# scale-lab/MTLoRA

Hardware: AMD Instinct MI355X
Metric: images/sec (train step) Swin-T/448 r=64 4-task (higher is better)
Workload: dtype bf16; 1 GPU; BASELINE configs[1]: Swin-T 448, 4 tasks (semseg,normals,sal,human_parts), r_shared=64 r_task=4 scale4; train step (fwd+loss+bwd+clip+AdamW), dropout .05, drop_path .2; per_gpu_batch=32, global_batch=32, img_size=448, parallelism=dp1, trainable_params=8344634, allreduce_bytes=0

## Files before the change

include/mtlora_hip.h:

```cpp
#ifndef MTLORA_HIP_H
#define MTLORA_HIP_H

#include <stdint.h>

#ifdef __cplusplus
extern "C" {
#endif

#define MTLORA_ABI_VERSION 9
#define MTLORA_MAX_TASKS 8

typedef enum mtlora_dtype {
    MTLORA_F32 = 0,
    MTLORA_BF16 = 1,
    MTLORA_F16 = 2
} mtlora_dtype;

typedef enum mtlora_status {
    MTLORA_OK = 0,
    MTLORA_ERR_DTYPE = -1,
    MTLORA_ERR_SHAPE = -2,
    MTLORA_ERR_ALIGN = -3,
    MTLORA_ERR_NULL = -4,
    MTLORA_ERR_WORKSPACE = -5,
    MTLORA_ERR_HIP = -6,
    MTLORA_ERR_UNSUPPORTED = -7
} mtlora_status;

int mtlora_version(void);
const char* mtlora_error_string(int status);

int mtlora_roll_and_window_partition_forward(const void* image, void* windows, int64_t B, int64_t H, int64_t W,
// ... 134 lines not shown
                                          void* const* d_branch, float* dgamma, float* dbeta, const float* scale, int64_t B,
                                          int64_t M, int64_t C, int x_dtype, int dy_dtype, void* scratch, int64_t scratch_bytes,
                                          const void* const* dx_addend, int merge_h, int merge_w, void* stream);

int mtlora_residual_layernorm_multi_fwd(int n, const void* shortcut, const void* const* branch, const float* scale, int64_t B,
                                        const float* gamma, const float* beta, void* const* x_new, void* const* y,
                                        float* const* mean, float* const* rstd, int64_t M, int64_t C, float eps, int x_dtype,
                                        int y_dtype, void* stream);
int mtlora_residual_layernorm_multi_bwd(int n, const void* const* dy, const void* const* x_new, const float* gamma,
                                        const float* const* mean, const float* const* rstd, const void* const* dx_addend,
                                        void* d_shortcut, void* const* d_branch, float* dgamma, float* dbeta, const float* scale,
                                        int64_t B, int64_t M, int64_t C, int x_dtype, int dy_dtype, void* scratch,
                                        int64_t scratch_bytes, void* stream);

int64_t mtlora_bn_scratch_bytes(int64_t R, int64_t C, int dtype);
int mtlora_bn_relu_fwd(const void* x, const float* gamma, const float* beta, float* running_mean, float* running_var,
                       float momentum, float eps, int relu, void* y, float* save_mean, float* save_rstd,
                       float* save_scale, float* save_shift, int64_t R, int64_t C, int dtype, void* scratch,
                       int64_t scratch_bytes, void* stream);
int mtlora_bn_relu_bwd(const void* dy, const void* x, const float* save_mean, const float* save_rstd,
                       const float* save_scale, const float* save_shift, int relu, void* dx, float* dgamma, float* dbeta,
                       int64_t R, int64_t C, int dtype, void* scratch, int64_t scratch_bytes, void* stream);

int mtlora_residual_droppath_fwd(int n, const void* const* res, const void* const* y, void* const* out,
                                 const float* scale, int64_t M, int64_t C, int64_t B, int res_dtype, int y_dtype,
                                 void* stream);
int mtlora_residual_droppath_bwd(int n, const void* const* g, void* const* dy, void* dres, const float* scale,
                                 int64_t M, int64_t C, int64_t B, int res_dtype, int y_dtype, void* stream);

int64_t mtlora_upsample_loss_partials(int64_t B, int h, int w, int scale);
int mtlora_upsample_loss(int kind, const void* low, const float* label, const float* stat, void* dlow, float* partials,
                         int64_t B, int h, int w, int C, int scale, int dtype, float ignore_index, void* stream);

int mtlora_upsample_metrics_sizes(int kind, int64_t B, int h, int w, int C, int scale, int64_t* n_int64,
                                  int64_t* n_float_partials);
int mtlora_upsample_metrics(int kind, const void* low, const float* label, const float* stat, int64_t* counts,
                            float* fpartials, int64_t B, int h, int w, int C, int scale, int dtype, float ignore_index,
                            void* stream);

int64_t mtlora_colsum_scratch_bytes(int64_t M, int64_t N);
int mtlora_colsum(const void* x, int64_t M, int64_t N, int dtype, float* out, void* scratch, int64_t scratch_bytes, void* stream);
int64_t mtlora_label_stat_scratch_bytes(int64_t n);
int mtlora_label_stat(const float* label, int64_t n, int kind, float ignore_index, float* out, void* scratch,
                      int64_t scratch_bytes, void* stream);

int mtlora_upsample_cl_fwd(const void* coarse, void* fine, int64_t B, int h, int w, int C, int scale, int64_t ld_fine,
// ... 68 lines not shown
```

mtlora_amd/_lib.py:

```python
from __future__ import annotations

import ctypes
import os
from ctypes import POINTER, Structure, c_char_p, c_float, c_int, c_int32, c_int64, c_uint64, c_void_p

import torch

MAX_TASKS = 8
ABI_VERSION = 9
F32, BF16, F16 = 0, 1, 2
_DT = {torch.float32: F32, torch.bfloat16: BF16, torch.float16: F16}

_HERE = os.path.dirname(os.path.abspath(__file__))
LIB_PATH = os.path.join(_HERE, "csrc", "libmtlora_hip.so")


class LinearDesc(Structure):
    _fields_ = [("M", c_int64), ("K", c_int64), ("N", c_int64), ("dtype", c_int32), ("mode", c_int32),
                ("T", c_int32), ("r_s", c_int32), ("r_t", c_int32 * MAX_TASKS), ("scale_s", c_float),
                ("scale_t", c_float * MAX_TASKS), ("has_x_tasks", c_int32), ("dropout_p", c_float),
                ("seed", c_uint64), ("seed_offset", c_void_p), ("bwd_phase", c_int32),
                ("sel_stream", c_int32), ("sel_dense", c_int32), ("sel_tn", c_int32), ("sel_projk", c_int32),
                ("max_cu", c_int32), ("packed", c_void_p),
                ("hid", c_int32), ("hid_pad_", c_int32), ("hid_ptr", c_void_p)]


HID_FWD_BASE, HID_P_GIVEN, HID_Q_GIVEN = 1, 2, 4


class AttnDesc(Structure):
    _fields_ = [("B", c_int64), ("H", c_int32), ("W", c_int32), ("window_size", c_int32), ("shift", c_int32),
                ("num_heads", c_int32), ("head_dim", c_int32), ("image_layout", c_int32), ("dtype", c_int32),
# ... 90 lines not shown
                                                      c_void_p]),
    "mtlora_residual_layernorm_streams_bwd": (c_int, [c_int, POINTER(c_void_p), POINTER(c_void_p), c_void_p, POINTER(c_void_p),
                                                      POINTER(c_void_p), POINTER(c_void_p), POINTER(c_void_p), c_void_p, c_void_p,
                                                      c_void_p, c_int64, c_int64, c_int64, c_int, c_int, c_void_p, c_int64,
                                                      POINTER(c_void_p), c_int, c_int, c_void_p]),
    "mtlora_residual_layernorm_multi_fwd": (c_int, [c_int, c_void_p, POINTER(c_void_p), c_void_p, c_int64, c_void_p, c_void_p,
                                                    POINTER(c_void_p), POINTER(c_void_p), POINTER(c_void_p), POINTER(c_void_p),
                                                    c_int64, c_int64, c_float, c_int, c_int, c_void_p]),
    "mtlora_residual_layernorm_multi_bwd": (c_int, [c_int, POINTER(c_void_p), POINTER(c_void_p), c_void_p, POINTER(c_void_p),
                                                    POINTER(c_void_p), POINTER(c_void_p), c_void_p, POINTER(c_void_p), c_void_p,
                                                    c_void_p, c_void_p, c_int64, c_int64, c_int64, c_int, c_int, c_void_p, c_int64,
                                                    c_void_p]),
    "mtlora_residual_layernorm_bwd": (c_int, [c_void_p, c_void_p, c_void_p, c_void_p, c_void_p, c_void_p, c_void_p, c_void_p,
                                              c_void_p, c_void_p, c_int64, c_int64, c_int64, c_int, c_int, c_void_p, c_int64,
                                              c_void_p, c_void_p]),
    "mtlora_layernorm_bwd": (c_int, [c_void_p, c_void_p, c_void_p, c_void_p, c_void_p, c_void_p, c_void_p, c_void_p,
                                     c_int64, c_int64, c_int, c_int, c_void_p, c_int64, c_void_p, c_int, c_int, c_void_p]),
    "mtlora_bn_scratch_bytes": (c_int64, [c_int64, c_int64, c_int]),
    "mtlora_bn_relu_fwd": (c_int, [c_void_p, c_void_p, c_void_p, c_void_p, c_void_p, c_float, c_float, c_int, c_void_p,
                                   c_void_p, c_void_p, c_void_p, c_void_p, c_int64, c_int64, c_int, c_void_p, c_int64,
                                   c_void_p]),
    "mtlora_bn_relu_bwd": (c_int, [c_void_p, c_void_p, c_void_p, c_void_p, c_void_p, c_void_p, c_int, c_void_p, c_void_p,
                                   c_void_p, c_int64, c_int64, c_int, c_void_p, c_int64, c_void_p]),
    "mtlora_residual_droppath_fwd": (c_int, [c_int, POINTER(c_void_p), POINTER(c_void_p), POINTER(c_void_p), c_void_p,
                                             c_int64, c_int64, c_int64, c_int, c_int, c_void_p]),
    "mtlora_residual_droppath_bwd": (c_int, [c_int, POINTER(c_void_p), POINTER(c_void_p), c_void_p, c_void_p, c_int64,
                                             c_int64, c_int64, c_int, c_int, c_void_p]),
    "mtlora_upsample_loss_partials": (c_int64, [c_int64, c_int, c_int, c_int]),
    "mtlora_colsum_scratch_bytes": (c_int64, [c_int64, c_int64]),
    "mtlora_colsum": (c_int, [c_void_p, c_int64, c_int64, c_int, c_void_p, c_void_p, c_int64, c_void_p]),
    "mtlora_label_stat_scratch_bytes": (c_int64, [c_int64]),
    "mtlora_label_stat": (c_int, [c_void_p, c_int64, c_int, c_float, c_void_p, c_void_p, c_int64, c_void_p]),
    "mtlora_upsample_loss": (c_int, [c_int, c_void_p, c_void_p, c_void_p, c_void_p, c_void_p, c_int64, c_int, c_int, c_int,
                                     c_int, c_int, ctypes.c_float, c_void_p]),
    "mtlora_upsample_metrics_sizes": (c_int, [c_int, c_int64, c_int, c_int, c_int, c_int, POINTER(c_int64), POINTER(c_int64)]),
    "mtlora_upsample_metrics": (c_int, [c_int, c_void_p, c_void_p, c_void_p, c_void_p, c_void_p, c_int64, c_int, c_int, c_int,
                                        c_int, c_int, ctypes.c_float, c_void_p]),
    "mtlora_upsample_cl_fwd": (c_int, [c_void_p, c_void_p, c_int64, c_int, c_int, c_int, c_int, c_int64, c_int, c_void_p]),
    "mtlora_upsample_cl_bwd": (c_int, [c_void_p, c_void_p, c_int64, c_int, c_int, c_int, c_int, c_int64, c_int, c_void_p]),
    "mtlora_block_save_bytes": (c_int64, [POINTER(BlockDesc)]),
    "mtlora_block_fwd_tmp_bytes": (c_int64, [POINTER(BlockDesc)]),
    "mtlora_block_bwd_scratch_bytes": (c_int64, [POINTER(BlockDesc)]),
    "mtlora_block_fwd": (c_int, [POINTER(BlockDesc), POINTER(BlockParams), c_void_p, c_void_p, c_void_p, c_void_p, c_void_p, c_int64,
                                 c_void_p, c_int64, c_void_p]),
    "mtlora_block_bwd": (c_int, [POINTER(BlockDesc), POINTER(BlockParams), c_void_p, c_void_p, c_void_p, c_void_p, c_void_p, c_void_p,
                                 c_int64, POINTER(BlockGrads), c_void_p, c_int64, c_int, c_void_p]),
# ... 84 lines not shown
```

mtlora_amd/csrc/build.py:

```python
import os
import subprocess
import sys
from concurrent.futures import ThreadPoolExecutor

HERE = os.path.dirname(os.path.abspath(__file__))
SOURCES = ["window_process.hip", "linear.hip", "attention.hip", "glue.hip", "loss.hip", "metrics.hip", "upsample.hip", "reduce.hip", "selftest.hip", "block.hip", "hid.hip"]
LIB = os.path.join(HERE, "libmtlora_hip.so")
FLAGS = ["--offload-arch=gfx950", "-O3", "-std=c++17", "-fPIC", "-Wno-unused-value", "-Wno-unused-result"]
if os.environ.get("MTLORA_ABLATE") == "1":
    FLAGS.append("-DMTL_NT_ABLATE=1")


def _hipcc():
    for c in (os.environ.get("HIPCC"), "/opt/rocm/bin/hipcc", "hipcc"):
        if c and (os.path.isabs(c) and os.path.exists(c) or not os.path.isabs(c)):
            return c
    return "hipcc"


def _stale(target, deps):
    if not os.path.exists(target):
        return True
    t = os.path.getmtime(target)
    return any(os.path.getmtime(d) > t for d in deps)


def build(force=False, verbose=True):
    hdrs = [os.path.join(HERE, f) for f in sorted(os.listdir(HERE)) if f.endswith(".h")]
    hdrs.append(os.path.join(HERE, "..", "..", "include", "mtlora_hip.h"))
# ... 25 lines not shown
```

mtlora_amd/csrc/glue.hip:

```cpp
#include "common.h"
#include "internal.h"

namespace {

constexpr int LN_MAXV = 8;

template <typename T>
__device__ __forceinline__ void ld_vec(const T* p, float (&f)[8]);
template <>
__device__ __forceinline__ void ld_vec<float>(const float* p, float (&f)[8]) {
    f32x4 v = *reinterpret_cast<const f32x4*>(p);
    f[0] = v[0];
    f[1] = v[1];
    f[2] = v[2];
    f[3] = v[3];
}
template <>
__device__ __forceinline__ void ld_vec<bf16>(const bf16* p, float (&f)[8]) {
    Vec16<bf16> v = mtl_ld16<bf16>(p);
#pragma unroll
    for (int e = 0; e < 8; ++e) f[e] = (float)v.e[e];
}
template <>
__device__ __forceinline__ void ld_vec<f16>(const f16* p, float (&f)[8]) {
// ... 1651 lines not shown
        MtlProfScope prof(PK_BN, (double)R * C * es * 2, s);
        if (dtype == MTLORA_F32)
            hipLaunchKernelGGL((k_bn_colsum<float, true>), dim3(p.nblk), dim3(threads), lds, s, p);
        else if (dtype == MTLORA_F16)
            hipLaunchKernelGGL((k_bn_colsum<f16, true>), dim3(p.nblk), dim3(threads), lds, s, p);
        else
            hipLaunchKernelGGL((k_bn_colsum<bf16, true>), dim3(p.nblk), dim3(threads), lds, s, p);
    }
    hipLaunchKernelGGL(k_bn_bwd_finalize, dim3((unsigned)mtl_ceil_div(C, 64)), dim3(64 * BN_FW), 0, s, p);
    {
        MtlProfScope prof(PK_BN, (double)R * C * es * 3, s);
        if (dtype == MTLORA_F32)
            hipLaunchKernelGGL((k_bn_apply<float, true>), dim3(apply_blocks), dim3(threads), 0, s, p);
        else if (dtype == MTLORA_F16)
            hipLaunchKernelGGL((k_bn_apply<f16, true>), dim3(apply_blocks), dim3(threads), 0, s, p);
        else
            hipLaunchKernelGGL((k_bn_apply<bf16, true>), dim3(apply_blocks), dim3(threads), 0, s, p);
    }
    MTL_CHECK_LAUNCH();
    return MTLORA_OK;
}
}

namespace {

struct ResParams {
    const void* res[MTLORA_MAX_TASKS + 1];
    const void* y[MTLORA_MAX_TASKS + 1];
    void* out[MTLORA_MAX_TASKS + 1];
    void* dres;
    const float* scale;
    int64_t M;
    int C, n, B;
    int64_t rows_per_sample;
};

template <typename TR, typename TY>
__global__ __launch_bounds__(256) void k_residual_fwd(const ResParams p) {
    const int64_t nvec = p.M * p.C / 8;
    const int k = blockIdx.y;
    const TR* res = reinterpret_cast<const TR*>(p.res[k]);
    const TY* y = reinterpret_cast<const TY*>(p.y[k]);
    TR* out = reinterpret_cast<TR*>(p.out[k]);
    for (int64_t i = (int64_t)blockIdx.x * 256 + threadIdx.x; i < nvec; i += (int64_t)gridDim.x * 256) {
        const int64_t row = (i * 8) / p.C;
        const float s = p.scale ? p.scale[(int64_t)k * p.B + row / p.rows_per_sample] : 1.f;
// ... 161 lines not shown
```

mtlora_amd/csrc/internal.h:

```cpp
#pragma once
#include <stdint.h>

#include "../../include/mtlora_hip.h"

#define MTL_INTERNAL extern "C" __attribute__((visibility("hidden")))

MTL_INTERNAL int mtli_layernorm_bwd(const void* dy, const void* x, const float* gamma, const float* mean, const float* rstd, void* dx,
                                    float* dgamma, float* dbeta, int64_t M, int64_t C, int x_dtype, int dy_dtype, void* scratch,
                                    int64_t scratch_bytes, const void* dx_addend, int phase, void* stream);
MTL_INTERNAL int mtli_residual_layernorm_bwd(const void* dy, const void* x_new, const float* gamma, const float* mean, const float* rstd,
                                             void* d_shortcut, void* d_branch, float* dgamma, float* dbeta, const float* scale,
                                             int64_t B, int64_t M, int64_t C, int x_dtype, int dy_dtype, void* scratch,
                                             int64_t scratch_bytes, const void* dx_addend, int phase, void* stream);

struct HidLaunch;
struct HidParams;
struct HidRedParams;
MTL_INTERNAL void mtli_hid_launch(const HidLaunch* L, const HidParams* q, void* stream);
MTL_INTERNAL void mtli_hid_rows_finish(int dtype, const float* rowpart, int n_chunk, int64_t M, int nt, const float* alpha, const int* off,
                                       void* out, int ldo, void* stream);
MTL_INTERNAL void mtli_hid_reduce(const HidRedParams* r, int64_t per, void* stream);
```

mtlora_amd/functional.py:

```python
from __future__ import annotations

import ctypes
import os
from dataclasses import dataclass, field
from typing import List, Optional, Sequence, Tuple

import torch

from . import _lib as L

_seed_counter = 0


_seed_offset: Optional[torch.Tensor] = None


def set_seed_offset(t: Optional[torch.Tensor]) -> None:
    global _seed_offset
    if t is not None and not (t.is_cuda and t.dtype == torch.int64 and t.numel() == 1):
        raise RuntimeError("mtlora_amd: the seed offset must be a CUDA int64 tensor with one element")
    _seed_offset = t


_factor_stream: Optional["torch.cuda.Stream"] = None
# ... 1115 lines not shown
                                    float(eps), int(relu), L.ptr(y), L.ptr(saves[0]), L.ptr(saves[1]), L.ptr(saves[2]),
                                    L.ptr(saves[3]), R, C, L.dtype_code(x), L.ptr(scratch), sb, L.stream_ptr())
        L.check(st, "mtlora_bn_relu_fwd")
        ctx.save_for_backward(x, saves)
        ctx.relu = relu
        return y

    @staticmethod
    def backward(ctx, dy):
        x, saves = ctx.saved_tensors
        R, C = x.shape
        dy = dy.to(x.dtype).contiguous()
        lib = L.lib()
        sb = lib.mtlora_bn_scratch_bytes(R, C, L.dtype_code(x))
        scratch = torch.empty(sb, dtype=torch.uint8, device=x.device)
        dx = torch.empty_like(x)
        dg = torch.empty(C, dtype=torch.float32, device=x.device)
        db = torch.empty(C, dtype=torch.float32, device=x.device)
        st = lib.mtlora_bn_relu_bwd(L.ptr(dy), L.ptr(x), L.ptr(saves[0]), L.ptr(saves[1]), L.ptr(saves[2]), L.ptr(saves[3]),
                                    int(ctx.relu), L.ptr(dx), L.ptr(dg), L.ptr(db), R, C, L.dtype_code(x), L.ptr(scratch), sb,
                                    L.stream_ptr())
        L.check(st, "mtlora_bn_relu_bwd")
        return dx, dg, db, None, None, None, None, None


class ResidualDropPathFn(torch.autograd.Function):

    @staticmethod
    def forward(ctx, scale, shared: bool, n: int, *tensors):
        nres = 1 if shared else n
        res, ys = list(tensors[:nres]), list(tensors[nres:nres + n])
        L.require_gpu(*res, *ys)
        B = res[0].shape[0]
        C = res[0].shape[-1]
        M = res[0].numel() // C
        res_c = [r.contiguous() for r in res]
        ys_c = [y.contiguous() for y in ys]
        outs = [torch.empty_like(res_c[0]) for _ in range(n)]
        rlist = res_c * n if shared else res_c
        st = L.lib().mtlora_residual_droppath_fwd(n, L.ptr_array9(rlist), L.ptr_array9(ys_c), L.ptr_array9(outs), L.ptr(scale),
                                                  M, C, B, L.dtype_code(res_c[0]), L.dtype_code(ys_c[0]), L.stream_ptr())
        L.check(st, "mtlora_residual_droppath_fwd")
        ctx.cfg = (shared, n, M, C, B, res_c[0].dtype, ys_c[0].dtype, res_c[0].shape)
        ctx.save_for_backward(scale)
        ctx.set_materialize_grads(False)
        return tuple(outs)
# ... 586 lines not shown
```

mtlora_amd/mtl_harness.py:

```python
from __future__ import annotations

import contextlib
import ctypes
import os
from typing import Dict, List, Mapping, Optional, Sequence

import torch
import torch.nn as nn
import torch.nn.functional as F

from . import functional as Fn
from .functional import BatchNormReluFn, UpsampleLossFn
from .lora import MTLoRALinear, mark_only_lora_as_trainable
from .swin_transformer_mtlora import SwinTransformerMTLoRA

NUM_OUTPUT = {"semseg": 21, "normals": 3, "sal": 1, "human_parts": 7, "depth": 1, "edge": 1}
EDGE_POS_WEIGHT = 0.95
NYUD4 = ("semseg", "depth", "normals", "edge")
NYUD_NUM_OUTPUT = {"semseg": 40}
LOSS_WEIGHTS = {"depth": 1.0, "semseg": 1.0, "human_parts": 2.0, "sal": 5.0, "edge": 50.0, "normals": 10.0}


def is_synthetic_task(t: str) -> bool:
    return len(t) >= 2 and t[0] == "t" and t[1:].isdigit()
# ... 69 lines not shown

def _streams_allowed() -> bool:
    return _GRAPH_STREAMS or not torch.cuda.is_current_stream_capturing()


class Downsampler(nn.Module):

    def __init__(self, dims, channels, input_res, bias=False, enabled=True):
        super().__init__()
        self.dims, self.input_res, self.enabled = dims, input_res, enabled
        if enabled:
            for i, (d, c) in enumerate(zip(dims, channels)):
                setattr(self, f"downsample_{i}", nn.Conv2d(d, c, 1, bias=bias))

    def forward(self, feats):
        maps = []
        for i, (f, r, d) in enumerate(zip(feats, self.input_res, self.dims)):
            if self.enabled:
                conv = getattr(self, f"downsample_{i}")
                B_, L_, _ = f.shape
                f = Fn.linear_big_m(f.reshape(B_ * L_, d), conv.weight.view(conv.out_channels, d), conv.bias).view(B_, L_, -1)
            maps.append(f.view(-1, r, r, f.shape[-1]).permute(0, 3, 1, 2))
        return maps


class HighResolutionHead(nn.Module):

    def __init__(self, backbone_channels, num_outputs):
        super().__init__()
        c = sum(backbone_channels)
        self.last_layer = nn.Sequential(nn.Conv2d(c, 4 * c, 1), nn.BatchNorm2d(4 * c, momentum=0.1),
                                        nn.ReLU(inplace=False), nn.Conv2d(4 * c, num_outputs, 1))

    def forward(self, x, channels_last_out: bool = False):
        B, _, Hh, Ww = x[0].shape
        c0, bn, _, c3 = self.last_layer
        w2d = c0.weight.view(c0.out_channels, c0.in_channels)
        xc = [m.permute(0, 2, 3, 1) for m in x]
        chans = [t.shape[3] for t in xc]
        if (x[0].is_cuda and all(t.is_contiguous() for t in xc) and all(c % 4 == 0 for c in chans[1:])
                and len({t.dtype for t in xc}) == 1 and xc[0].dtype in (torch.float32, torch.bfloat16)
                and all(Hh % t.shape[1] == 0 and Ww % t.shape[2] == 0 and Hh // t.shape[1] == Ww // t.shape[2] for t in xc)):
            t = Fn.ConcatUpsampleFn.apply(*xc)
            offs, ld = Fn.ConcatUpsampleFn.layout(chans)
            col_idx = None
            if ld != w2d.shape[1]:
                key = (tuple(offs), tuple(chans), w2d.device)
                if getattr(self, "_col_key", None) != key:
                    self._col_idx = torch.cat([torch.arange(o, o + c) for o, c in zip(offs, chans)]).to(w2d.device)
                    self._col_key = key
                col_idx = self._col_idx
        else:
            cat = torch.cat([x[0]] + [F.interpolate(m, (Hh, Ww), mode="bilinear") for m in x[1:]], 1)
            t = cat.permute(0, 2, 3, 1).reshape(B * Hh * Ww, cat.shape[1])
            col_idx = None
        h = Fn.linear_big_m(t, w2d, c0.bias, feeds_batchnorm=bn.training, col_index=col_idx)
        if bn.training and bn.track_running_stats and bn.num_batches_tracked is not None:
            bn.num_batches_tracked.add_(1)
        if bn.training and h.is_cuda and h.dtype in (torch.float32, torch.bfloat16, torch.float16) and h.shape[1] % 8 == 0:
            h = BatchNormReluFn.apply(h, bn.weight, bn.bias, bn.running_mean, bn.running_var, bn.momentum, bn.eps,
                                      getattr(self, "relu", True))
        else:
            h = F.batch_norm(h, bn.running_mean, bn.running_var, bn.weight, bn.bias, bn.training or not bn.track_running_stats,
                             bn.momentum, bn.eps)
            if getattr(self, "relu", True):
                h = F.relu(h)
        w3, b3, nc = c3.weight.view(c3.out_channels, c3.in_channels), c3.bias, c3.out_channels
        o = Fn.linear_big_m(h, w3, b3, pad_rows=(8 - nc % 8) if (h.is_cuda and nc % 8) else 0)
        o = (o if o.shape[1] == nc else o[:, :nc].contiguous()).view(B, Hh, Ww, nc)
        return o if channels_last_out else o.permute(0, 3, 1, 2)


class DecoderGroup(nn.Module):
    def __init__(self, tasks, num_outputs, channels, out_size):
        super().__init__()
        self.tasks, self.out_size = tasks, out_size
        self.decoders = nn.ModuleDict({t: HighResolutionHead(channels, num_outputs[t]) for t in tasks})

    def forward(self, x, upsample: bool = True, tasks=None):
        tasks = self.tasks if tasks is None else tasks
        if not upsample:
            return {t: self.decoders[t](x[t], channels_last_out=True) for t in tasks}
        return {t: F.interpolate(self.decoders[t](x[t]), self.out_size, mode="bilinear") for t in tasks}


class MultiTaskSwin(nn.Module):

    def __init__(self, backbone: SwinTransformerMTLoRA, tasks: Sequence[str], num_outputs: Mapping[str, int] = NUM_OUTPUT,
                 decoder_channels=(18, 36, 72, 144)):
        super().__init__()
# ... 423 lines not shown
```

Before: 1156 images/sec.

## Fuse head BatchNorm+ReLU with final 1x1 conv into custom MFMA kernels

Adds a fused head-tail path that computes BN statistics, then applies BN+ReLU on the fly while doing the small final projection with MFMA, so the normalized activation is never written out. Backward is split into a stats kernel (dgamma/dbeta, dW3, db3, BN correction terms) and an apply kernel that recomputes the BN+ReLU output and produces dz directly. This is meant to remove the materialized BN output tensor and its extra read/write traffic at large M (B*448*448/16 rows with 4C channels). It adds new kernels with per-wave slab loops and grid capped at the CU count, and it falls back to the old path when hooks are present or shapes are unsupported.

Result: slower. 1126 images/sec (-2.6%).

```diff
diff --git a/include/mtlora_hip.h b/include/mtlora_hip.h
--- a/include/mtlora_hip.h
+++ b/include/mtlora_hip.h
@@ -7,7 +7,7 @@
 extern "C" {
 #endif
 
-#define MTLORA_ABI_VERSION 9
+#define MTLORA_ABI_VERSION 10
 #define MTLORA_MAX_TASKS 8
 
 typedef enum mtlora_dtype {
@@ -188,6 +188,16 @@
                        const float* save_scale, const float* save_shift, int relu, void* dx, float* dgamma, float* dbeta,
                        int64_t R, int64_t C, int dtype, void* scratch, int64_t scratch_bytes, void* stream);
 
+int64_t mtlora_head_tail_scratch_bytes(int64_t R, int64_t C, int nc, int dtype);
+int mtlora_head_tail_fwd(const void* h, const float* gamma, const float* beta, float* running_mean, float* running_var,
+                         float momentum, float eps, int relu, const void* w3, const float* b3, void* o, float* save, int64_t R,
+                         int64_t C, int nc, int dtype, void* scratch, int64_t scratch_bytes, void* stream);
+int mtlora_head_tail_bwd_stats(const void* dout, const void* h, const void* w3, const float* save, int relu, float* dgamma,
+                               float* dbeta, float* cmean, float* dw3, float* db3, int64_t R, int64_t C, int nc, int dtype,
+                               void* scratch, int64_t scratch_bytes, void* stream);
+int mtlora_head_tail_bwd_apply(const void* dout, const void* h, const void* w3, const float* save, const float* cmean, int relu,
+                               void* dz, int64_t R, int64_t C, int nc, int dtype, void* stream);
+
 int mtlora_residual_droppath_fwd(int n, const void* const* res, const void* const* y, void* const* out,
                                  const float* scale, int64_t M, int64_t C, int64_t B, int res_dtype, int y_dtype,
                                  void* stream);
diff --git a/mtlora_amd/_lib.py b/mtlora_amd/_lib.py
--- a/mtlora_amd/_lib.py
+++ b/mtlora_amd/_lib.py
@@ -7,7 +7,7 @@
 import torch
 
 MAX_TASKS = 8
-ABI_VERSION = 9
+ABI_VERSION = 10
 F32, BF16, F16 = 0, 1, 2
 _DT = {torch.float32: F32, torch.bfloat16: BF16, torch.float16: F16}
 
@@ -144,6 +144,13 @@
                                    c_void_p]),
     "mtlora_bn_relu_bwd": (c_int, [c_void_p, c_void_p, c_void_p, c_void_p, c_void_p, c_void_p, c_int, c_void_p, c_void_p,
                                    c_void_p, c_int64, c_int64, c_int, c_void_p, c_int64, c_void_p]),
+    "mtlora_head_tail_scratch_bytes": (c_int64, [c_int64, c_int64, c_int, c_int]),
+    "mtlora_head_tail_fwd": (c_int, [c_void_p, c_void_p, c_void_p, c_void_p, c_void_p, c_float, c_float, c_int, c_void_p, c_void_p,
+                                     c_void_p, c_void_p, c_int64, c_int64, c_int, c_int, c_void_p, c_int64, c_void_p]),
+    "mtlora_head_tail_bwd_stats": (c_int, [c_void_p, c_void_p, c_void_p, c_void_p, c_int, c_void_p, c_void_p, c_void_p, c_void_p,
+                                           c_void_p, c_int64, c_int64, c_int, c_int, c_void_p, c_int64, c_void_p]),
+    "mtlora_head_tail_bwd_apply": (c_int, [c_void_p, c_void_p, c_void_p, c_void_p, c_void_p, c_int, c_void_p, c_int64, c_int64,
+                                           c_int, c_int, c_void_p]),
     "mtlora_residual_droppath_fwd": (c_int, [c_int, POINTER(c_void_p), POINTER(c_void_p), POINTER(c_void_p), c_void_p,
                                              c_int64, c_int64, c_int64, c_int, c_int, c_void_p]),
     "mtlora_residual_droppath_bwd": (c_int, [c_int, POINTER(c_void_p), POINTER(c_void_p), c_void_p, c_void_p, c_int64,
diff --git a/mtlora_amd/csrc/build.py b/mtlora_amd/csrc/build.py
--- a/mtlora_amd/csrc/build.py
+++ b/mtlora_amd/csrc/build.py
@@ -4,7 +4,7 @@
 from concurrent.futures import ThreadPoolExecutor
 
 HERE = os.path.dirname(os.path.abspath(__file__))
-SOURCES = ["window_process.hip", "linear.hip", "attention.hip", "glue.hip", "loss.hip", "metrics.hip", "upsample.hip", "reduce.hip", "selftest.hip", "block.hip", "hid.hip"]
+SOURCES = ["window_process.hip", "linear.hip", "attention.hip", "glue.hip", "loss.hip", "metrics.hip", "upsample.hip", "reduce.hip", "selftest.hip", "block.hip", "hid.hip", "head.hip"]
 LIB = os.path.join(HERE, "libmtlora_hip.so")
 FLAGS = ["--offload-arch=gfx950", "-O3", "-std=c++17", "-fPIC", "-Wno-unused-value", "-Wno-unused-result"]
 if os.environ.get("MTLORA_ABLATE") == "1":
diff --git a/mtlora_amd/csrc/glue.hip b/mtlora_amd/csrc/glue.hip
--- a/mtlora_amd/csrc/glue.hip
+++ b/mtlora_amd/csrc/glue.hip
@@ -1697,6 +1697,64 @@
 }
 }
 
+int mtli_bn_stats_fwd(const void* x, const float* gamma, const float* beta, float* running_mean, float* running_var, float momentum,
+                      float eps, float* save_mean, float* save_rstd, float* save_scale, float* save_shift, int64_t R, int64_t C,
+                      int dtype, void* scratch, int64_t scratch_bytes, void* stream) {
+    BnParams p = {};
+    int st = bn_setup(p, R, C, dtype);
+    if (st != MTLORA_OK) return st;
+    if (scratch_bytes < (int64_t)p.nblk * 2 * C * 4) return MTLORA_ERR_WORKSPACE;
+    p.x = x;
+    p.gamma = gamma;
+    p.beta = beta;
+    p.running_mean = running_mean;
+    p.running_var = running_var;
+    p.mean = save_mean;
+    p.rstd = save_rstd;
+    p.scale = save_scale;
+    p.shift = save_shift;
+    p.part = reinterpret_cast<float*>(scratch);
+    p.momentum = momentum;
+    p.eps = eps;
+    hipStream_t s = (hipStream_t)stream;
+    const int threads = (int)mtl_round_up((int64_t)p.rows_per_iter * p.VW, 64);
+    const size_t lds = (size_t)p.rows_per_iter * 2 * C * 4;
+    {
+        MtlProfScope prof(PK_BN, (double)R * C * mtl_elem_size(dtype), s);
+        if (dtype == MTLORA_F16)
+            hipLaunchKernelGGL((k_bn_colsum<f16, false>), dim3(p.nblk), dim3(threads), lds, s, p);
+        else if (dtype == MTLORA_BF16)
+            hipLaunchKernelGGL((k_bn_colsum<bf16, false>), dim3(p.nblk), dim3(threads), lds, s, p);
+        else
+            return MTLORA_ERR_DTYPE;
+    }
+    hipLaunchKernelGGL(k_bn_finalize, dim3((unsigned)mtl_ceil_div(C, 64)), dim3(64 * BN_FW), 0, s, p);
+    MTL_CHECK_LAUNCH();
+    return MTLORA_OK;
+}
+
+int64_t mtli_bn_stats_scratch_bytes(int64_t R, int64_t C, int dtype) {
+    BnParams p = {};
+    if (bn_setup(p, R, C, dtype) != MTLORA_OK) return -1;
+    return (int64_t)p.nblk * 2 * C * 4;
+}
+
+int mtli_bn_bwd_finalize(const float* part, int nblk, int64_t R, int64_t C, float* dgamma, float* dbeta, float* c1, float* c2,
+                         void* stream) {
+    BnParams p = {};
+    p.part = const_cast<float*>(part);
+    p.nblk = nblk;
+    p.R = R;
+    p.C = (int)C;
+    p.dgamma = dgamma;
+    p.dbeta = dbeta;
+    p.c1 = c1;
+    p.c2 = c2;
+    hipLaunchKernelGGL(k_bn_bwd_finalize, dim3((unsigned)mtl_ceil_div(C, 64)), dim3(64 * BN_FW), 0, (hipStream_t)stream, p);
+    MTL_CHECK_LAUNCH();
+    return MTLORA_OK;
+}
+
 namespace {
 
 struct ResParams {
diff --git a/mtlora_amd/csrc/head.hip b/mtlora_amd/csrc/head.hip
--- /dev/null
+++ b/mtlora_amd/csrc/head.hip
@@ -0,0 +1,536 @@
+#include "common.h"
+#include "internal.h"
+#include <atomic>
+
+namespace {
+
+constexpr int HT_WAVES = 8;
+constexpr int HT_LDS_MAX = 160 * 1024;
+constexpr int HT_MAX_PARTS = 256;
+
+struct HtParams {
+    const void* h;
+    const void* w3;
+    const void* dout;
+    void* o;
+    void* dz;
+    const float* b3;
+    const float* mean;
+    const float* rstd;
+    const float* scale;
+    const float* shift;
+    const float* c1;
+    const float* c2;
+    float* part_bn;
+    float* part_w;
+    float* part_b;
+    float* dw3;
+    float* db3;
+    int64_t R;
+    int C, nc, relu, n_slabs, parts;
+};
+
+template <typename T>
+__device__ __forceinline__ void ht_mma(const u32x4& a, const u32x4& b, f32x16& c) {
+    if constexpr (__is_same(T, f16))
+        c = __builtin_amdgcn_mfma_f32_32x32x16_f16(__builtin_bit_cast(f16x8, a), __builtin_bit_cast(f16x8, b), c, 0, 0, 0);
+    else
+        c = __builtin_amdgcn_mfma_f32_32x32x16_bf16(__builtin_bit_cast(bf16x8, a), __builtin_bit_cast(bf16x8, b), c, 0, 0, 0);
+}
+
+template <typename T>
+__device__ __forceinline__ float ht_cvt(uint32_t bits) {
+    if constexpr (__is_same(T, f16))
+        return (float)__builtin_bit_cast(f16, (uint16_t)bits);
+    else
+        return __builtin_bit_cast(float, bits << 16);
+}
+
+__device__ __forceinline__ u32x4 ht_w3_col(const uint16_t* w3, int C, int nc, int n0, int c) {
+    uint32_t v[8];
+#pragma unroll
+    for (int k = 0; k < 8; ++k) v[k] = (c < C && n0 + k < nc) ? (uint32_t)w3[(int64_t)(n0 + k) * C + c] : 0u;
+    return u32x4{v[0] | (v[1] << 16), v[2] | (v[3] << 16), v[4] | (v[5] << 16), v[6] | (v[7] << 16)};
+}
+
+__device__ __forceinline__ u32x4 ht_do_row(const uint16_t* d, int64_t m, int64_t R, int nc, int n0) {
+    uint32_t v[8];
+#pragma unroll
+    for (int k = 0; k < 8; ++k) v[k] = (m < R && n0 + k < nc) ? (uint32_t)d[m * nc + n0 + k] : 0u;
+    return u32x4{v[0] | (v[1] << 16), v[2] | (v[3] << 16), v[4] | (v[5] << 16), v[6] | (v[7] << 16)};
+}
+
+template <typename T>
+__global__ __launch_bounds__(64 * HT_WAVES) void k_ht_fwd(const HtParams p) {
+    extern __shared__ __attribute__((aligned(16))) unsigned char smem[];
+    const int tid = threadIdx.x, lane = tid & 63, wave = tid >> 6, hh = lane >> 5, rl = lane & 31;
+    const int C = p.C, nc = p.nc, NG = (C + 63) >> 6, Cp = NG * 64;
+    u32x4* wl = reinterpret_cast<u32x4*>(smem);
+    float* ssc = reinterpret_cast<float*>(smem + (size_t)NG * 4096);
+    float* ssh = ssc + Cp;
+    const T* w3 = reinterpret_cast<const T*>(p.w3);
+    for (int f = tid; f < NG * 256; f += 64 * HT_WAVES) {
+        const int s = f >> 6, l = f & 63, n = l & 31, col = 64 * (s >> 2) + 32 * (l >> 5) + 8 * (s & 3);
+        wl[f] = (n < nc && col < C) ? *reinterpret_cast<const u32x4*>(w3 + (int64_t)n * C + col) : u32x4{0u, 0u, 0u, 0u};
+    }
+    for (int c = tid; c < Cp; c += 64 * HT_WAVES) {
+        ssc[c] = c < C ? p.scale[c] : 0.f;
+        ssh[c] = c < C ? p.shift[c] : 0.f;
+    }
+    __syncthreads();
+    const T* h = reinterpret_cast<const T*>(p.h);
+    T* o = reinterpret_cast<T*>(p.o);
+    const bool relu = p.relu != 0;
+    for (int slab = blockIdx.x * HT_WAVES + wave; slab < p.n_slabs; slab += gridDim.x * HT_WAVES) {
+        const int64_t m = (int64_t)slab * 32 + rl;
+        const bool ok = m < p.R;
+        const T* row = h + (ok ? m : 0) * C;
+        f32x16 acc;
+#pragma unroll
+        for (int r = 0; r < 16; ++r) acc[r] = 0.f;
+        for (int g = 0; g < NG; ++g) {
+            const int cb = 64 * g + 32 * hh;
+            u32x4 raw[4];
+#pragma unroll
+            for (int j = 0; j < 4; ++j)
+                raw[j] = (ok && cb + 8 * j < C) ? *reinterpret_cast<const u32x4*>(row + cb + 8 * j) : u32x4{0u, 0u, 0u, 0u};
+#pragma unroll
+            for (int j = 0; j < 4; ++j) {
+                const int col = cb + 8 * j;
+                const f32x4 s0 = *reinterpret_cast<const f32x4*>(ssc + col), s1 = *reinterpret_cast<const f32x4*>(ssc + col + 4);
+                const f32x4 t0 = *reinterpret_cast<const f32x4*>(ssh + col), t1 = *reinterpret_cast<const f32x4*>(ssh + col + 4);
+                const float sc[8] = {s0[0], s0[1], s0[2], s0[3], s1[0], s1[1], s1[2], s1[3]};
+                const float sh[8] = {t0[0], t0[1], t0[2], t0[3], t1[0], t1[1], t1[2], t1[3]};
+                u32x4 b;
+#pragma unroll
+                for (int q = 0; q < 4; ++q) {
+                    float y0 = mtl_lo2<T>(raw[j][q]) * sc[2 * q] + sh[2 * q];
+                    float y1 = mtl_hi2<T>(raw[j][q]) * sc[2 * q + 1] + sh[2 * q + 1];
+                    y0 = (relu && y0 < 0.f) ? 0.f : y0;
+                    y1 = (relu && y1 < 0.f) ? 0.f : y1;
+                    b[q] = mtl_pk2<T>(y0, y1);
+                }
+                ht_mma<T>(wl[(4 * g + j) * 64 + lane], b, acc);
+            }
+        }
+        if (ok) {
+#pragma unroll
+            for (int r = 0; r < 16; ++r) {
+                const int n = 8 * (r >> 2) + 4 * hh + (r & 3);
+                if (n < nc) o[m * nc + n] = mtl_from_f32<T>(acc[r] + (p.b3 ? p.b3[n] : 0.f));
+            }
+        }
+    }
+}
+
+template <typename T>
+__global__ __launch_bounds__(64 * HT_WAVES) void k_ht_bwd_apply(const HtParams p) {
+    extern __shared__ __attribute__((aligned(16))) unsigned char smem[];
+    const int tid = threadIdx.x, lane = tid & 63, wave = tid >> 6, hh = lane >> 5, rl = lane & 31;
+    const int C = p.C, nc = p.nc, NG = (C + 63) >> 6, Cp = NG * 64;
+    u32x4* wt = reinterpret_cast<u32x4*>(smem);
+    f32x4* cst = reinterpret_cast<f32x4*>(smem + (size_t)NG * 4096);
+    const uint16_t* w3 = reinterpret_cast<const uint16_t*>(p.w3);
+    for (int f = tid; f < NG * 256; f += 64 * HT_WAVES) {
+        const int g = f >> 8, b = (f >> 7) & 1, s = (f >> 6) & 1, l = f & 63, i = l & 31;
+        const int c = 64 * g + 32 * ((i >> 2) & 1) + 16 * b + 4 * (i >> 3) + (i & 3);
+        wt[f] = ht_w3_col(w3, C, nc, 16 * s + 8 * (l >> 5), c);
+    }
+    for (int c = tid; c < Cp; c += 64 * HT_WAVES) {
+        f32x4 v = {0.f, 0.f, 0.f, 0.f};
+        if (c < C) {
+            const float sc = p.scale[c], t = sc * p.c2[c] * p.rstd[c];
+            v = f32x4{sc, p.shift[c], -t, t * p.mean[c] - sc * p.c1[c]};
+        }
+        cst[c] = v;
+    }
+    __syncthreads();
+    const T* h = reinterpret_cast<const T*>(p.h);
+    T* dz = reinterpret_cast<T*>(p.dz);
+    const uint16_t* dout = reinterpret_cast<const uint16_t*>(p.dout);
+    const bool relu = p.relu != 0;
+    for (int slab = blockIdx.x * HT_WAVES + wave; slab < p.n_slabs; slab += gridDim.x * HT_WAVES) {
+        const int64_t m = (int64_t)slab * 32 + rl;
+        const bool ok = m < p.R;
+        const int64_t rowoff = (ok ? m : 0) * C;
+        u32x4 dof[2];
+#pragma unroll
+        for (int s = 0; s < 2; ++s) dof[s] = ht_do_row(dout, m, p.R, nc, 16 * s + 8 * hh);
+        for (int g = 0; g < NG; ++g) {
+            const int cb = 64 * g + 32 * hh;
+            u32x4 raw[4];
+#pragma unroll
+            for (int j = 0; j < 4; ++j)
+                raw[j] = (ok && cb + 8 * j < C) ? *reinterpret_cast<const u32x4*>(h + rowoff + cb + 8 * j) : u32x4{0u, 0u, 0u, 0u};
+            f32x16 acc[2];
+#pragma unroll
+            for (int b = 0; b < 2; ++b) {
+#pragma unroll
+                for (int r = 0; r < 16; ++r) acc[b][r] = 0.f;
+#pragma unroll
+                for (int s = 0; s < 2; ++s) ht_mma<T>(wt[((g * 2 + b) * 2 + s) * 64 + lane], dof[s], acc[b]);
+            }
+#pragma unroll
+            for (int j = 0; j < 4; ++j) {
+                const int col = cb + 8 * j;
+                u32x4 out;
+#pragma unroll
+                for (int q = 0; q < 4; ++q) {
+                    float v[2];
+#pragma unroll
+                    for (int e = 0; e < 2; ++e) {
+                        const int k = 2 * q + e;
+                        const f32x4 cs = cst[col + k];
+                        const float x = e ? mtl_hi2<T>(raw[j][q]) : mtl_lo2<T>(raw[j][q]);
+                        const float yv = x * cs[0] + cs[1];
+                        const float gm = (relu && yv <= 0.f) ? 0.f : acc[j >> 1][8 * (j & 1) + k];
+                        v[e] = cs[0] * gm + cs[2] * x + cs[3];
+                    }
+                    out[q] = mtl_pk2<T>(v[0], v[1]);
+                }
+                if (ok && col < C) *reinterpret_cast<u32x4*>(dz + rowoff + col) = out;
+            }
+        }
+    }
+}
+
+template <typename T, int NBW>
+__global__ __launch_bounds__(64 * HT_WAVES) void k_ht_bwd_stats(const HtParams p) {
+    extern __shared__ __attribute__((aligned(16))) unsigned char smem[];
+    const int tid = threadIdx.x, lane = tid & 63, wave = tid >> 6, hh = lane >> 5, rl = lane & 31;
+    const int C = p.C, nc = p.nc, nblk = (C + 31) >> 5;
+    u32x4* wf = reinterpret_cast<u32x4*>(smem);
+    const uint16_t* w3 = reinterpret_cast<const uint16_t*>(p.w3);
+    for (int f = tid; f < nblk * 128; f += 64 * HT_WAVES) {
+        const int blk = f >> 7, s = (f >> 6) & 1, l = f & 63;
+        wf[f] = ht_w3_col(w3, C, nc, 16 * s + 8 * (l >> 5), 32 * blk + (l & 31));
+    }
+    __syncthreads();
+    float sc[NBW], sh[NBW], mu[NBW], rs[NBW], s0[NBW], s1[NBW];
+    f32x16 dw[NBW], dbacc;
+#pragma unroll
+    for (int j = 0; j < NBW; ++j) {
+        const int c = 32 * (wave + HT_WAVES * j) + rl;
+        const bool cok = c < C;
+        sc[j] = cok ? p.scale[c] : 0.f;
+        sh[j] = cok ? p.shift[c] : 0.f;
+        mu[j] = cok ? p.mean[c] : 0.f;
+        rs[j] = cok ? p.rstd[c] : 0.f;
+        s0[j] = s1[j] = 0.f;
+#pragma unroll
+        for (int r = 0; r < 16; ++r) dw[j][r] = 0.f;
+    }
+#pragma unroll
+    for (int r = 0; r < 16; ++r) dbacc[r] = 0.f;
+    const uint32_t one2 = mtl_pk2<T>(1.f, 1.f);
+    const u32x4 ones = {one2, one2, one2, one2};
+    const uint16_t* hu = reinterpret_cast<const uint16_t*>(p.h);
+    const uint16_t* dout = reinterpret_cast<const uint16_t*>(p.dout);
+    const bool relu = p.relu != 0;
+    const int64_t R = p.R;
+    for (int slab = blockIdx.x; slab < p.n_slabs; slab += gridDim.x) {
+        const int64_t m0 = (int64_t)slab * 32;
+        u32x4 dor[2], dot[2];
+#pragma unroll
+        for (int s = 0; s < 2; ++s) {
+            dor[s] = ht_do_row(dout, m0 + rl, R, nc, 16 * s + 8 * hh);
+            uint32_t v[8];
+#pragma unroll
+            for (int k = 0; k < 8; ++k) {
+                const int64_t m = m0 + 16 * s + 8 * (k >> 2) + 4 * hh + (k & 3);
+                v[k] = (rl < nc && m < R) ? (uint32_t)dout[m * nc + rl] : 0u;
+            }
+            dot[s] = u32x4{v[0] | (v[1] << 16), v[2] | (v[3] << 16), v[4] | (v[5] << 16), v[6] | (v[7] << 16)};
+        }
+        if (wave == 0) {
+#pragma unroll
+            for (int s = 0; s < 2; ++s) ht_mma<T>(dot[s], ones, dbacc);
+        }
+#pragma unroll
+        for (int j = 0; j < NBW; ++j) {
+            const int blk = wave + HT_WAVES * j;
+            if (blk < nblk) {
+                const int c = 32 * blk + rl;
+                const bool cok = c < C;
+                uint32_t hx[16];
+#pragma unroll
+                for (int r = 0; r < 16; ++r) {
+                    const int64_t m = m0 + 8 * (r >> 2) + 4 * hh + (r & 3);
+                    hx[r] = (cok && m < R) ? (uint32_t)hu[m * C + c] : 0u;
+                }
+                f32x16 g;
+#pragma unroll
+                for (int r = 0; r < 16; ++r) g[r] = 0.f;
+#pragma unroll
+                for (int s = 0; s < 2; ++s) ht_mma<T>(dor[s], wf[(blk * 2 + s) * 64 + lane], g);
+                float yr[16];
+#pragma unroll
+                for (int r = 0; r < 16; ++r) {
+                    const float x = ht_cvt<T>(hx[r]);
+                    const float yv = x * sc[j] + sh[j];
+                    const float gm = (relu && yv <= 0.f) ? 0.f : g[r];
+                    s0[j] += gm;
+                    s1[j] += gm * (x - mu[j]) * rs[j];
+                    yr[r] = (relu && yv < 0.f) ? 0.f : yv;
+                }
+#pragma unroll
+                for (int s = 0; s < 2; ++s) {
+                    const u32x4 yb = {mtl_pk2<T>(yr[8 * s + 0], yr[8 * s + 1]), mtl_pk2<T>(yr[8 * s + 2], yr[8 * s + 3]),
+                                      mtl_pk2<T>(yr[8 * s + 4], yr[8 * s + 5]), mtl_pk2<T>(yr[8 * s + 6], yr[8 * s + 7])};
+                    ht_mma<T>(dot[s], yb, dw[j]);
+                }
+            }
+        }
+    }
+    const int64_t b = blockIdx.x;
+#pragma unroll
+    for (int j = 0; j < NBW; ++j) {
+        const int blk = wave + HT_WAVES * j;
+        const int c = 32 * blk + rl;
+        const float a0 = s0[j] + __shfl_xor(s0[j], 32), a1 = s1[j] + __shfl_xor(s1[j], 32);
+        if (blk < nblk && c < C) {
+            if (hh == 0) {
+                p.part_bn[(b * 2 + 0) * C + c] = a0;
+                p.part_bn[(b * 2 + 1) * C + c] = a1;
+            }
+#pragma unroll
+            for (int r = 0; r < 16; ++r) {
+                const int n = 8 * (r >> 2) + 4 * hh + (r & 3);
+                if (n < nc) p.part_w[(b * nc + n) * C + c] = dw[j][r];
+            }
+        }
+    }
+    if (wave == 0 && rl == 0) {
+#pragma unroll
+        for (int r = 0; r < 16; ++r) p.part_b[b * 32 + 8 * (r >> 2) + 4 * hh + (r & 3)] = dbacc[r];
+    }
+}
+
+__global__ __launch_bounds__(256) void k_ht_combine(const HtParams p) {
+    __shared__ float sm[4][64];
+    const int l = threadIdx.x & 63, g = threadIdx.x >> 6;
+    const int64_t nw = (int64_t)p.nc * p.C, total = nw + p.nc;
+    const int64_t e = (int64_t)blockIdx.x * 64 + l;
+    float s = 0.f;
+    if (e < total) {
+        const float* src = e < nw ? p.part_w + e : p.part_b + (e - nw);
+        const int64_t stride = e < nw ? nw : 32;
+#pragma unroll 4
+        for (int b = g; b < p.parts; b += 4) s += src[b * stride];
+    }
+    sm[g][l] = s;
+    __syncthreads();
+    if (g == 0 && e < total) {
+        const float t = ((sm[0][l] + sm[1][l]) + sm[2][l]) + sm[3][l];
+        if (e < nw)
+            p.dw3[e] = t;
+        else
+            p.db3[e - nw] = t;
+    }
+}
+
+int num_cu() {
+    static std::atomic<int> cache{0};
+    int cu = cache.load(std::memory_order_relaxed);
+    if (cu == 0) {
+        int dev = 0;
+        cu = 256;
+        if (hipGetDevice(&dev) != hipSuccess || hipDeviceGetAttribute(&cu, hipDeviceAttributeMultiprocessorCount, dev) != hipSuccess ||
+            cu <= 0) {
+            (void)hipGetLastError();
+            cu = 256;
+        }
+        cache.store(cu, std::memory_order_relaxed);
+    }
+    return cu;
+}
+
+template <typename K>
+void raise_lds(K kernel, size_t bytes) {
+    static std::atomic<unsigned long long> done{0};
+    if (bytes <= 48 * 1024) return;
+    int dev = 0;
+    if (hipGetDevice(&dev) != hipSuccess) dev = 0;
+    if ((done.load(std::memory_order_relaxed) >> (dev & 63)) & 1ull) return;
+    if (hipFuncSetAttribute((const void*)kernel, hipFuncAttributeMaxDynamicSharedMemorySize, HT_LDS_MAX) != hipSuccess) {
+        (void)hipGetLastError();
+        return;
+    }
+    done.fetch_or(1ull << (dev & 63), std::memory_order_relaxed);
+}
+
+struct HtGeom {
+    int n_slabs, NG, nblk, nbw, parts;
+    size_t lds_fwd, lds_apply, lds_stats;
+};
+
+int ht_setup(HtGeom& g, int64_t R, int64_t C, int nc, int dtype) {
+    if (dtype != MTLORA_BF16 && dtype != MTLORA_F16) return MTLORA_ERR_DTYPE;
+    if (R <= 0 || C <= 0 || C % 8 || nc < 1 || nc > 32) return MTLORA_ERR_SHAPE;
+    if (C > 32 * HT_WAVES * 5 || R > ((int64_t)1 << 36)) return MTLORA_ERR_UNSUPPORTED;
+    g.n_slabs = (int)mtl_ceil_div(R, 32);
+    g.NG = (int)mtl_ceil_div(C, 64);
+    g.nblk = (int)mtl_ceil_div(C, 32);
+    const int need = (int)mtl_ceil_div(g.nblk, HT_WAVES);
+    g.nbw = need <= 1 ? 1 : need <= 2 ? 2 : need <= 3 ? 3 : 5;
+    g.parts = g.n_slabs < HT_MAX_PARTS ? g.n_slabs : HT_MAX_PARTS;
+    g.lds_fwd = (size_t)g.NG * 4096 + (size_t)g.NG * 64 * 8;
+    g.lds_apply = (size_t)g.NG * 4096 + (size_t)g.NG * 64 * 16;
+    g.lds_stats = (size_t)g.nblk * 2048;
+    if (g.lds_apply > (size_t)HT_LDS_MAX) return MTLORA_ERR_UNSUPPORTED;
+    return MTLORA_OK;
+}
+
+int64_t ht_bwd_floats(const HtGeom& g, int64_t C, int nc) { return (int64_t)g.parts * (2 * C + (int64_t)nc * C + 32); }
+
+}
+
+extern "C" {
+
+int64_t mtlora_head_tail_scratch_bytes(int64_t R, int64_t C, int nc, int dtype) {
+    HtGeom g;
+    if (ht_setup(g, R, C, nc, dtype) != MTLORA_OK) return -1;
+    const int64_t fwd = mtli_bn_stats_scratch_bytes(R, C, dtype);
+    if (fwd < 0) return -1;
+    const int64_t bwd = ht_bwd_floats(g, C, nc) * 4;
+    return (fwd > bwd ? fwd : bwd) + 256;
+}
+
+int mtlora_head_tail_fwd(const void* h, const float* gamma, const float* beta, float* running_mean, float* running_var,
+                         float momentum, float eps, int relu, const void* w3, const float* b3, void* o, float* saves, int64_t R,
+                         int64_t C, int nc, int dtype, void* scratch, int64_t scratch_bytes, void* stream) {
+    HtGeom g;
+    int st = ht_setup(g, R, C, nc, dtype);
+    if (st != MTLORA_OK) return st;
+    if (!h || !gamma || !beta || !w3 || !o || !saves || !scratch) return MTLORA_ERR_NULL;
+    if (((uintptr_t)h | (uintptr_t)w3 | (uintptr_t)scratch) & 15u) return MTLORA_ERR_ALIGN;
+    st = mtli_bn_stats_fwd(h, gamma, beta, running_mean, running_var, momentum, eps, saves, saves + C, saves + 2 * C, saves + 3 * C, R, C,
+                           dtype, scratch, scratch_bytes, stream);
+    if (st != MTLORA_OK) return st;
+    HtParams p = {};
+    p.h = h;
+    p.w3 = w3;
+    p.b3 = b3;
+    p.o = o;
+    p.scale = saves + 2 * C;
+    p.shift = saves + 3 * C;
+    p.R = R;
+    p.C = (int)C;
+    p.nc = nc;
+    p.relu = relu;
+    p.n_slabs = g.n_slabs;
+    hipStream_t s = (hipStream_t)stream;
+    const int64_t want = mtl_ceil_div(g.n_slabs, HT_WAVES), cap = 2 * (int64_t)num_cu();
+    const unsigned grid = (unsigned)(want < cap ? want : cap);
+    MtlProfScope prof(PK_BN, (double)R * C * 2, s);
+    if (dtype == MTLORA_F16) {
+        raise_lds(k_ht_fwd<f16>, g.lds_fwd);
+        hipLaunchKernelGGL((k_ht_fwd<f16>), dim3(grid), dim3(64 * HT_WAVES), g.lds_fwd, s, p);
+    } else {
+        raise_lds(k_ht_fwd<bf16>, g.lds_fwd);
+        hipLaunchKernelGGL((k_ht_fwd<bf16>), dim3(grid), dim3(64 * HT_WAVES), g.lds_fwd, s, p);
+    }
+    MTL_CHECK_LAUNCH();
+    return MTLORA_OK;
+}
+
+int mtlora_head_tail_bwd_stats(const void* dout, const void* h, const void* w3, const float* saves, int relu, float* dgamma,
+                               float* dbeta, float* cmean, float* dw3, float* db3, int64_t R, int64_t C, int nc, int dtype,
+                               void* scratch, int64_t scratch_bytes, void* stream) {
+    HtGeom g;
+    int st = ht_setup(g, R, C, nc, dtype);
+    if (st != MTLORA_OK) return st;
+    if (!dout || !h || !w3 || !saves || !dgamma || !dbeta || !cmean || !dw3 || !db3 || !scratch) return MTLORA_ERR_NULL;
+    if (((uintptr_t)h | (uintptr_t)scratch) & 15u) return MTLORA_ERR_ALIGN;
+    if (scratch_bytes < ht_bwd_floats(g, C, nc) * 4) return MTLORA_ERR_WORKSPACE;
+    HtParams p = {};
+    p.h = h;
+    p.w3 = w3;
+    p.dout = dout;
+    p.mean = saves;
+    p.rstd = saves + C;
+    p.scale = saves + 2 * C;
+    p.shift = saves + 3 * C;
+    p.part_bn = reinterpret_cast<float*>(scratch);
+    p.part_w = p.part_bn + (int64_t)g.parts * 2 * C;
+    p.part_b = p.part_w + (int64_t)g.parts * nc * C;
+    p.dw3 = dw3;
+    p.db3 = db3;
+    p.R = R;
+    p.C = (int)C;
+    p.nc = nc;
+    p.relu = relu;
+    p.n_slabs = g.n_slabs;
+    p.parts = g.parts;
+    hipStream_t s = (hipStream_t)stream;
+    {
+        MtlProfScope prof(PK_BN, (double)R * C * 2, s);
+#define HT_STATS(TT, NB)                                                                                              \
+    do {                                                                                                              \
+        raise_lds(k_ht_bwd_stats<TT, NB>, g.lds_stats);                                                               \
+        hipLaunchKernelGGL((k_ht_bwd_stats<TT, NB>), dim3(g.parts), dim3(64 * HT_WAVES), g.lds_stats, s, p);          \
+    } while (0)
+#define HT_STATS_T(TT)            \
+    do {                          \
+        if (g.nbw == 1)           \
+            HT_STATS(TT, 1);      \
+        else if (g.nbw == 2)      \
+            HT_STATS(TT, 2);      \
+        else if (g.nbw == 3)      \
+            HT_STATS(TT, 3);      \
+        else                      \
+            HT_STATS(TT, 5);      \
+    } while (0)
+        if (dtype == MTLORA_F16)
+            HT_STATS_T(f16);
+        else
+            HT_STATS_T(bf16);
+#undef HT_STATS_T
+#undef HT_STATS
+    }
+    MTL_CHECK_LAUNCH();
+    st = mtli_bn_bwd_finalize(p.part_bn, g.parts, R, C, dgamma, dbeta, cmean, cmean + C, stream);
+    if (st != MTLORA_OK) return st;
+    hipLaunchKernelGGL(k_ht_combine, dim3((unsigned)mtl_ceil_div((int64_t)nc * C + nc, 64)), dim3(256), 0, s, p);
+    MTL_CHECK_LAUNCH();
+    return MTLORA_OK;
+}
+
+int mtlora_head_tail_bwd_apply(const void* dout, const void* h, const void* w3, const float* saves, const float* cmean, int relu,
+                               void* dz, int64_t R, int64_t C, int nc, int dtype, void* stream) {
+    HtGeom g;
+    int st = ht_setup(g, R, C, nc, dtype);
+    if (st != MTLORA_OK) return st;
+    if (!dout || !h || !w3 || !saves || !cmean || !dz) return MTLORA_ERR_NULL;
+    if (((uintptr_t)h | (uintptr_t)dz) & 15u) return MTLORA_ERR_ALIGN;
+    HtParams p = {};
+    p.h = h;
+    p.w3 = w3;
+    p.dout = dout;
+    p.dz = dz;
+    p.mean = saves;
+    p.rstd = saves + C;
+    p.scale = saves + 2 * C;
+    p.shift = saves + 3 * C;
+    p.c1 = cmean;
+    p.c2 = cmean + C;
+    p.R = R;
+    p.C = (int)C;
+    p.nc = nc;
+    p.relu = relu;
+    p.n_slabs = g.n_slabs;
+    hipStream_t s = (hipStream_t)stream;
+    const int64_t want = mtl_ceil_div(g.n_slabs, HT_WAVES), cap = num_cu();
+    const unsigned grid = (unsigned)(want < cap ? want : cap);
+    MtlProfScope prof(PK_BN, (double)R * C * 4, s);
+    if (dtype == MTLORA_F16) {
+        raise_lds(k_ht_bwd_apply<f16>, g.lds_apply);
+        hipLaunchKernelGGL((k_ht_bwd_apply<f16>), dim3(grid), dim3(64 * HT_WAVES), g.lds_apply, s, p);
+    } else {
+        raise_lds(k_ht_bwd_apply<bf16>, g.lds_apply);
+        hipLaunchKernelGGL((k_ht_bwd_apply<bf16>), dim3(grid), dim3(64 * HT_WAVES), g.lds_apply, s, p);
+    }
+    MTL_CHECK_LAUNCH();
+    return MTLORA_OK;
+}
+}
diff --git a/mtlora_amd/csrc/internal.h b/mtlora_amd/csrc/internal.h
--- a/mtlora_amd/csrc/internal.h
+++ b/mtlora_amd/csrc/internal.h
@@ -13,6 +13,13 @@
                                              int64_t B, int64_t M, int64_t C, int x_dtype, int dy_dtype, void* scratch,
                                              int64_t scratch_bytes, const void* dx_addend, int phase, void* stream);
 
+MTL_INTERNAL int64_t mtli_bn_stats_scratch_bytes(int64_t R, int64_t C, int dtype);
+MTL_INTERNAL int mtli_bn_stats_fwd(const void* x, const float* gamma, const float* beta, float* running_mean, float* running_var,
+                                   float momentum, float eps, float* save_mean, float* save_rstd, float* save_scale, float* save_shift,
+                                   int64_t R, int64_t C, int dtype, void* scratch, int64_t scratch_bytes, void* stream);
+MTL_INTERNAL int mtli_bn_bwd_finalize(const float* part, int nblk, int64_t R, int64_t C, float* dgamma, float* dbeta, float* c1,
+                                      float* c2, void* stream);
+
 struct HidLaunch;
 struct HidParams;
 struct HidRedParams;
diff --git a/mtlora_amd/functional.py b/mtlora_amd/functional.py
--- a/mtlora_amd/functional.py
+++ b/mtlora_amd/functional.py
@@ -1161,6 +1161,68 @@
                                     L.stream_ptr())
         L.check(st, "mtlora_bn_relu_bwd")
         return dx, dg, db, None, None, None, None, None
+
+
+HEAD_TAIL_FUSED = os.environ.get("MTLORA_HEAD_TAIL", "1") != "0"
+
+
+def head_tail_ok(h: torch.Tensor, nc: int) -> bool:
+    return (HEAD_TAIL_FUSED and h.is_cuda and h.dim() == 2 and h.dtype in (torch.bfloat16, torch.float16)
+            and h.shape[1] % 8 == 0 and h.shape[1] <= 1280 and 1 <= nc <= 32 and h.shape[0] >= 1)
+
+
+class HeadTailFn(torch.autograd.Function):
+
+    @staticmethod
+    def forward(ctx, h, bn_weight, bn_bias, running_mean, running_var, momentum: float, eps: float, w3, b3, relu: bool):
+        L.require_gpu(h, bn_weight, bn_bias, w3, b3)
+        R, C = h.shape
+        nc = w3.shape[0]
+        h = h.contiguous()
+        g, b = bn_weight.detach().float().contiguous(), bn_bias.detach().float().contiguous()
+        w = w3.detach().to(h.dtype).contiguous()
+        b3f = None if b3 is None else b3.detach().float().contiguous()
+        o = torch.empty((R, nc), dtype=h.dtype, device=h.device)
+        saves = torch.empty(4, C, dtype=torch.float32, device=h.device)
+        lib = L.lib()
+        code = L.dtype_code(h)
+        sb = lib.mtlora_head_tail_scratch_bytes(R, C, nc, code)
+        if sb < 0:
+            raise RuntimeError(f"mtlora_amd: unsupported head-tail shape ({R}, {C}) -> {nc} {h.dtype}")
+        scratch = torch.empty(sb, dtype=torch.uint8, device=h.device)
+        st = lib.mtlora_head_tail_fwd(L.ptr(h), L.ptr(g), L.ptr(b), L.ptr(running_mean), L.ptr(running_var), float(momentum), float(eps),
+                                      int(relu), L.ptr(w), L.ptr(b3f), L.ptr(o), L.ptr(saves), R, C, nc, code, L.ptr(scratch), sb,
+                                      L.stream_ptr())
+        L.check(st, "mtlora_head_tail_fwd")
+        ctx.save_for_backward(h, saves, w)
+        ctx.cfg = (bool(relu), bn_weight.dtype, bn_bias.dtype, w3.dtype, None if b3 is None else b3.dtype)
+        return o
+
+    @staticmethod
+    def backward(ctx, do):
+        h, saves, w = ctx.saved_tensors
+        relu, gdt, bdt, wdt, b3dt = ctx.cfg
+        R, C = h.shape
+        nc = w.shape[0]
+        do = do.to(h.dtype).contiguous()
+        lib = L.lib()
+        code = L.dtype_code(h)
+        sb = lib.mtlora_head_tail_scratch_bytes(R, C, nc, code)
+        scratch = torch.empty(sb, dtype=torch.uint8, device=h.device)
+        f32 = dict(dtype=torch.float32, device=h.device)
+        dg, db, cmean = torch.empty(C, **f32), torch.empty(C, **f32), torch.empty(2, C, **f32)
+        dw3, db3 = torch.empty(nc, C, **f32), torch.empty(nc, **f32)
+        st = lib.mtlora_head_tail_bwd_stats(L.ptr(do), L.ptr(h), L.ptr(w), L.ptr(saves), int(relu), L.ptr(dg), L.ptr(db), L.ptr(cmean),
+                                            L.ptr(dw3), L.ptr(db3), R, C, nc, code, L.ptr(scratch), sb, L.stream_ptr())
+        L.check(st, "mtlora_head_tail_bwd_stats")
+        dz = None
+        if ctx.needs_input_grad[0]:
+            dz = torch.empty_like(h)
+            st = lib.mtlora_head_tail_bwd_apply(L.ptr(do), L.ptr(h), L.ptr(w), L.ptr(saves), L.ptr(cmean), int(relu), L.ptr(dz), R, C,
+                                                nc, code, L.stream_ptr())
+            L.check(st, "mtlora_head_tail_bwd_apply")
+        return (dz, dg.to(gdt), db.to(bdt), None, None, None, None, dw3.to(wdt),
+                None if b3dt is None else db3.to(b3dt), None)
 
 
 class ResidualDropPathFn(torch.autograd.Function):
diff --git a/mtlora_amd/mtl_harness.py b/mtlora_amd/mtl_harness.py
--- a/mtlora_amd/mtl_harness.py
+++ b/mtlora_amd/mtl_harness.py
@@ -115,6 +115,10 @@
                 f = Fn.linear_big_m(f.reshape(B_ * L_, d), conv.weight.view(conv.out_channels, d), conv.bias).view(B_, L_, -1)
             maps.append(f.view(-1, r, r, f.shape[-1]).permute(0, 3, 1, 2))
         return maps
+
+
+def _hooked(seq: nn.Module) -> bool:
+    return any(m._forward_hooks or m._forward_pre_hooks or m._backward_hooks or m._backward_pre_hooks for m in (seq, *seq))
 
 
 class HighResolutionHead(nn.Module):
@@ -150,6 +154,11 @@
         h = Fn.linear_big_m(t, w2d, c0.bias, feeds_batchnorm=bn.training, col_index=col_idx)
         if bn.training and bn.track_running_stats and bn.num_batches_tracked is not None:
             bn.num_batches_tracked.add_(1)
+        w3, b3, nc = c3.weight.view(c3.out_channels, c3.in_channels), c3.bias, c3.out_channels
+        if bn.training and bn.affine and bn.momentum is not None and Fn.head_tail_ok(h, nc) and not _hooked(self.last_layer):
+            o = Fn.HeadTailFn.apply(h, bn.weight, bn.bias, bn.running_mean, bn.running_var, bn.momentum, bn.eps, w3, b3,
+                                    getattr(self, "relu", True)).view(B, Hh, Ww, nc)
+            return o if channels_last_out else o.permute(0, 3, 1, 2)
         if bn.training and h.is_cuda and h.dtype in (torch.float32, torch.bfloat16, torch.float16) and h.shape[1] % 8 == 0:
             h = BatchNormReluFn.apply(h, bn.weight, bn.bias, bn.running_mean, bn.running_var, bn.momentum, bn.eps,
                                       getattr(self, "relu", True))
@@ -158,7 +167,6 @@
                              bn.momentum, bn.eps)
             if getattr(self, "relu", True):
                 h = F.relu(h)
-        w3, b3, nc = c3.weight.view(c3.out_channels, c3.in_channels), c3.bias, c3.out_channels
         o = Fn.linear_big_m(h, w3, b3, pad_rows=(8 - nc % 8) if (h.is_cuda and nc % 8) else 0)
         o = (o if o.shape[1] == nc else o[:, :nc].contiguous()).view(B, Hh, Ww, nc)
         return o if channels_last_out else o.permute(0, 3, 1, 2)
```
